# thanosDelatolas/eva-vos

Hardware: AMD Instinct MI355X
Metric: frames/sec STCN mask-propagate 480p 1-obj (higher is better)
Workload: dtype f32; 1 GPU; DAVIS-17-val-shaped 480x854 (padded 480x864) single-object STCN propagate: fresh engine, interact(mask,0), T=66 frames/video, mem_freq=5, top_k=50; one video per step per GPU; videos_per_gpu=38, streams_per_gpu=4, key_lookahead=0, clips=8 distinct synthetic clips (one per pooled engine), weights=synthetic recipe seed 0 (no checkpoints offline)

## Files before the change

### eva_vos_amd/_lib.py

```python
from __future__ import annotations

import ctypes as C
import os

import torch

_HERE = os.path.dirname(os.path.abspath(__file__))
LIB_PATH = os.environ.get("STCN_LIB") or os.path.join(_HERE, "libstcn_hip.so")

K_CLASSES = ("conv", "conv_reduce", "memread", "elementwise", "conv_n1", "other", "wino_input", "fusion_conv", "attention")


class WeightDesc(C.Structure):
    _fields_ = [("name", C.c_char_p), ("data", C.c_void_p), ("ndim", C.c_int32), ("shape", C.c_int64 * 4)]


class EngineOpts(C.Structure):
    _fields_ = [(n, C.c_int32) for n in ("lookahead", "decode_batch", "key_batch", "fuse_side")]


class ModelOpts(C.Structure):
    _fields_ = [("top_k", C.c_int32), ("km", C.c_float)]


# ... 24 lines not shown
    "stcn_engine_create_ex": (_I, [_P, _I, _I, _I, _I, _I, _P, _P, _P, _P, C.POINTER(EngineOpts), C.POINTER(_P)]),
    "stcn_engine_get_opts": (_I, [_P, C.POINTER(EngineOpts)]),
    "stcn_engine_destroy": (_I, [_P]),
    "stcn_engine_reset": (_I, [_P]),
    "stcn_engine_clone": (_I, [_P, _P, _P, _P, C.POINTER(_P)]),
    "stcn_interact": (_I, [_P, _P, _I, _I, _I]),
    "stcn_get_stats": (_I, [_P, C.POINTER(Stats)]),
    "stcn_get_flops": (_I, [_P, C.POINTER(_D)]),
    "stcn_last_conv_path": (C.c_char_p, []),
    "stcn_test_conv_trace": (_I, [_I]),
    "stcn_test_conv_trace_get": (C.c_char_p, []),
    "stcn_test_conv": (_I, [_P, _P, _P, _P, _P, _P] + [_I] * 11),
    "stcn_test_conv_ex": (_I, [_P, _P, _P, _P, _P, _P] + [_I] * 11 + [_P, _I, _L, _L, _L, _I, _L]),
    "stcn_test_conv_path": (_I, [_I] * 9 + [C.c_char_p, _I]),
    "stcn_test_conv_plan": (_I, [_I] * 9 + [C.POINTER(C.c_int32), _I, C.POINTER(_D)]),
    "stcn_test_sweep_plan": (_I, [_I, _I, _I, _I, C.POINTER(C.c_int32), _I, C.POINTER(C.c_int32)]),
    "stcn_test_encode_key": (_I, [_P, _P, _P, _I, _I, _P, _P, _P, _P, _P]),
    "stcn_test_encode_value": (_I, [_P, _P, _P, _P, _P, _I, _I, _I, _P]),
    "stcn_test_memory_read": (_I, [_P, _P, _P, _P, _I, _I, _I, _P, _P, _P]),
    "stcn_test_memory_read_k": (_I, [_P, _P, _P, _P, _I, _I, _I, _I, _P, _P, _P]),
    "stcn_test_memory_read_km": (_I, [_P, _P, _P, _P, _I, _I, _I, _I, _I, _I, _F, _P, _P, _P, _P]),
    "stcn_bench_memory_read": (_I, [_P, _P, _P, _P, _I, _I, _I, _I, _P, C.POINTER(_F), C.POINTER(C.c_int32)]),
    "stcn_bench_memory_read_k": (_I, [_P, _P, _P, _P, _I, _I, _I, _I, _I, _P, C.POINTER(_F), C.POINTER(C.c_int32)]),
    "stcn_bench_memory_read_km": (_I, [_P, _P, _P, _P, _I, _I, _I, _I, _I, _I, _F, _I, _P, C.POINTER(_F), C.POINTER(C.c_int32)]),
    "stcn_memread_plan": (_I, [_I, _I, C.POINTER(C.c_int32)]),
    "stcn_memread_scratch": (_I, [_I, C.POINTER(C.c_int64)]),
    "stcn_test_kernel": (_I, [C.c_char_p, _P, C.POINTER(_P), _I, C.POINTER(C.c_int64), _I, C.POINTER(_D), _I]),
    "stcn_test_fail_at": (_I, [_I]),
    "stcn_test_side_delay_us": (_I, [_I]),
    "stcn_test_decode": (_I, [_P, _P, _P, _P, _P, _P, _I, _I, _I, _P, _P]),
# ... 57 lines not shown
```

### eva_vos_amd/csrc/engine.cpp

```cpp
#include "engine.h"
#include "src_hash.h"

#include <algorithm>
#include <atomic>
#include <cmath>
#include <cstdarg>
#include <cstdio>
#include <cstdlib>
#include <cstring>
#include <map>
#include <mutex>
#include <unordered_map>
#include <utility>

namespace stcn {

static thread_local char g_err[512] = "";
void set_error(const char *fmt, ...) {
    va_list ap;
    va_start(ap, fmt);
    vsnprintf(g_err, sizeof(g_err), fmt, ap);
    va_end(ap);
}
const char *get_error() { return g_err; }

Knobs Knobs::from_env() {
    Knobs k;
    k.wino_min_cin = env_int("STCN_WINO_MIN_CIN", k.wino_min_cin);
    k.wino_ppw = env_int("STCN_WINO_PPW", k.wino_ppw);
    k.wino4_chunk_mb = env_int("STCN_WINO4_CHUNK_MB", k.wino4_chunk_mb);
    k.fusion_conv12 = env_int("STCN_FUSION_CONV12", k.fusion_conv12) != 0;
    k.fusion_wino = env_int("STCN_FUSION_WINO", k.fusion_wino) != 0;
    k.pw_chain = env_int("STCN_PW_CHAIN", k.pw_chain);
    return k;
}

void Prof::reset() {
    for (int i = 0; i < STCN_K_COUNT; ++i) { flops[i] = 0; bytes[i] = 0; exec_flops[i] = 0; launches[i] = 0; }
    hbm_conv_flops = hbm_conv_bytes = hbm_conv_ms = 0; hbm_conv_launches = 0;
    wino2_flops = wino4_flops = 0;
    for (auto &e : events) { pool.push_back(e.a); pool.push_back(e.b); }
    events.clear();
}
Prof::Ev &Prof::push_pair(int cls, bool hbm) {
    Ev e; e.cls = cls; e.hbm = hbm;
    for (hipEvent_t *p : {&e.a, &e.b}) {
        if (!pool.empty()) { *p = pool.back(); pool.pop_back(); }
        else (void)hipEventCreate(p);
// ... 74 lines not shown
int make_wino_fusion12(Model &m, ConvW &cw, const std::vector<float> &w) {
    if (!wants_wino_fusion12(cw)) return STCN_OK;
    std::vector<float> w16((size_t)32 * 9 * 16, 0.f), u((size_t)16 * 16 * 32);
    for (int n = 0; n < 32; ++n)
        for (int tap = 0; tap < 9; ++tap)
            for (int c = 0; c < 12; ++c) w16[((size_t)n * 9 + tap) * 16 + c] = w[(size_t)n * cw.Kp + tap * 12 + c];
    wino_transform_weights(w16.data(), 32, 16, 9 * 16, u.data());
    return upload(m, u, &cw.wino_u);
}

int make_wino4(Model &m, ConvW &cw, const std::vector<float> &w) {
    if (!wants_wino4(cw)) return STCN_OK;
    std::vector<float> u((size_t)36 * cw.cin_p * cw.cout);
    wino4_transform_weights(w.data(), cw.cout, cw.cin_p, cw.Kp, u.data());
    return upload(m, u, &cw.wino4_u);
}

static bool wino4_layer(const std::string &name) {
    if (name == "value_encoder.layer2.0.conv1" || name == "value_encoder.layer3.0.conv1") return false;
    if (name == "key_encoder.layer2.0.conv2" || name == "key_encoder.layer3.0.conv2") return false;
    static const bool key_f4 = env_on("STCN_WINO4_KEY");
    if (key_f4 && name.compare(0, 12, "key_encoder.") == 0 && name.size() > 6 && name.compare(name.size() - 6, 6, ".conv2") == 0) return true;
    static const bool kproj_f4 = env_on("STCN_WINO4_KEYPROJ");
    if (kproj_f4 && name == "key_proj.key_proj") return true;
    return name.compare(0, 8, "decoder.") == 0 || name == "key_comp" || name.compare(0, 20, "value_encoder.fuser.") == 0 ||
           name.compare(0, 19, "value_encoder.layer") == 0;
}

static std::vector<float> repack(const HostT &wt, const std::vector<float> &scale, int lo, int hi, const ConvW &cw) {
    const int cout = (int)wt.sh[0], cin = (int)wt.sh[1], kh = (int)wt.sh[2], kw = (int)wt.sh[3];
// ... 30 lines not shown
                const float sc = g[n] / std::sqrt(var[n] + 1e-5f);
                scale[n] = sc;
                bias[n] = (bias[n] - mu[n]) * sc + b[n];
            }
        }
        ConvW cw;
        cw.cout = cout; cw.cin = cin; cw.kh = kh; cw.kw = kw;
        cw.cin_p = (cin + 3) / 4 * 4;
        cw.K = kh * kw * cw.cin_p;
        cw.Kp = (cw.K + 31) / 32 * 32;
        const std::vector<float> w = repack(wt, scale, 0, cin, cw);
        int rc = upload(m, w, &cw.w);
        if (rc) return rc;
        rc = upload(m, bias, &cw.bias);
        if (rc) return rc;
        if ((rc = make_wino(m, cw, w)) || (rc = make_wino_fusion12(m, cw, w))) return rc;
        if (wino4_layer(pre) && (rc = make_wino4(m, cw, w))) return rc;
        cw.bias0 = bias[0];
        m.conv[pre] = cw;
        static const struct { const char *name; int c0; } splits[] = {
            {"decoder.compress.conv1", 512}, {"decoder.compress.downsample", 512},
            {"value_encoder.fuser.block1.conv1", 256}, {"value_encoder.fuser.block1.downsample", 256}};
        for (const auto &sp : splits) {
            if (pre != sp.name) continue;
            for (int part = 0; part < 2; ++part) {
                const int lo = part ? sp.c0 : 0, hi = part ? cin : sp.c0;
                ConvW pw;
                pw.cout = cout; pw.cin = hi - lo; pw.cin_p = hi - lo; pw.kh = kh; pw.kw = kw;
                pw.K = kh * kw * pw.cin_p; pw.Kp = (pw.K + 31) / 32 * 32;
                const std::vector<float> ww = repack(wt, scale, lo, hi, pw);
                std::vector<float> bb = part ? bias : std::vector<float>(cout, 0.f);
// ... 230 lines not shown
namespace {
struct ConvPathRec {
    ConvPlan plan{};
    char lit[96] = "";
};
thread_local ConvPathRec g_path;
thread_local char g_path_str[96] = "";
thread_local bool g_trace_on = false;
thread_local std::string g_trace;
}
const char *format_conv_path(const ConvPlan &pl, char *out, size_t n) {
    switch (pl.family) {
    case CONV_FUSION: snprintf(out, n, "%s", pl.fusion_wino ? "fusion_wino" : "fusion_direct"); break;
    case CONV_WINO4: snprintf(out, n, "wino4 chunks=%d%s", pl.w4.chunks, pl.reduce ? " +tail" : ""); break;
    case CONV_WINO2: snprintf(out, n, "wino2 ppw=%d splitk=%d", pl.ppw, pl.splitk); break;
    case CONV_DIRECT: snprintf(out, n, "%s%s splitk=%d", pl.variant, pl.tail ? " +tail" : "", pl.splitk); break;
    default: snprintf(out, n, "%s", "");
    }
    return out;
}
const char *last_conv_path() { return g_path.plan.family == CONV_LITERAL ? g_path.lit : format_conv_path(g_path.plan, g_path_str, sizeof(g_path_str)); }
void set_conv_path(const char *s) { g_path.plan.family = CONV_LITERAL; snprintf(g_path.lit, sizeof(g_path.lit), "%s", s); }
void conv_trace(int on) { g_trace_on = on != 0; if (on) g_trace.clear(); }
const char *conv_trace_get() { return g_trace.c_str(); }

int plan_conv(const Model &m, const Work &w, const std::string &name, const ConvArgs &a, ConvP &p, ConvPlan &pl) {
    auto it = m.conv.find(name);
    if (it == m.conv.end()) { set_error("missing conv '%s'", name.c_str()); return STCN_E_MISSING; }
    const ConvW &cw = it->second;
    const int B = a.B, H = a.H, W = a.W, c0 = a.c0, c1 = a.c1;
// ... 60 lines not shown
            eg[c] = w.prof->attach(cls, hbm_acc);
            if (c < pl.n_in) ei[c] = w.prof->attach(STCN_K_WINO_INPUT);
        }
        if (pl.reduce) er = w.prof->attach(STCN_K_CONV_REDUCE);
    }
    if (g_trace_on) { char b[96]; g_trace += name; g_trace += '='; g_trace += format_conv_path(pl, b, sizeof(b)); g_trace += '\n'; }
    switch (pl.family) {
    case CONV_FUSION: fusion_conv_launch(p, pl, s, eg[0]); break;
    case CONV_WINO4: wino4_launch(p, pl, w.wino_v, s, ei, eg, er); break;
    case CONV_WINO2: wino_launch(p, pl, w.wino_v, s, ei[0], eg[0], er); break;
    default: conv_launch(p, s, eg[0], er);
    }
    return launch_status(name.c_str());
}

#define RC(x) do { int rc_ = (x); if (rc_) return rc_; } while (0)

int encode_key(const Model &m, Work &w, hipStream_t s, const float *img4, const KeyOut &o, int B, long out_bs) {
    const Dims &d = w.d;
    const long obs = B > 1 ? out_bs : 0;
    const long ibs = obs ? obs : CONV_DENSE;
    RC(run_conv(m, w, s, "key_encoder.conv1", ConvArgs(img4, 4, B, d.nh, d.nw).strided(2).out(w.A).relu(0, 1)));
    { Scope sc(w.prof, STCN_K_ELEMWISE, s); maxpool3x3s2_launch(w.A, w.B, B, d.h2, d.w2, 64, s); }
    struct St { const char *name; int n, planes, stride; } stages[3] = {{"res2", 3, 64, 1}, {"layer2", 4, 128, 2}, {"layer3", 6, 256, 2}};
    int H = d.h4, W = d.w4, cin = 64;
    float *x = w.B;
    for (int si = 0; si < 3; ++si) {
        const St &st = stages[si];
        for (int i = 0; i < st.n; ++i) {
            const std::string p = std::string("key_encoder.") + st.name + "." + std::to_string(i);
            const int sd = i == 0 ? st.stride : 1;
            const int OH = H / sd, OW = W / sd;
            const float *idt = x;
            if (i == 0) { RC(run_conv(m, w, s, p + ".downsample.0", ConvArgs(x, cin, B, H, W).strided(sd).out(w.D))); idt = w.D; }
            RC(run_conv(m, w, s, p + ".conv1", ConvArgs(x, cin, B, H, W).out(w.C).relu(0, 1)));
            RC(run_conv(m, w, s, p + ".conv2", ConvArgs(w.C, st.planes, B, H, W).strided(sd).out(w.A).relu(0, 1)));
            float *dst = x;
            long dst_bs = 0;
// ... 48 lines not shown
    const ConvArgs in = ConvArgs(x0, c0, B, H, W, bs0).concat(x1, c1, bs1);
    const float *skip; long skip_bs;
    if (m.conv.count(p + ".downsample")) {
        RC(run_conv(m, w, s, p + ".downsample", ConvArgs(in).out(t2)));
        skip = t2; skip_bs = CONV_DENSE;
    } else { skip = x0; skip_bs = bs0; }
    RC(run_conv(m, w, s, p + ".conv1", ConvArgs(in).out(t1).relu(1, 1)));
    RC(run_conv(m, w, s, p + ".conv2", ConvArgs(t1, cw.cout, B, H, W).out(out, out_bs).residual(skip, skip_bs)));
    return STCN_OK;
}

int encode_value(const Model &m, Work &w, hipStream_t s, const float *img4, const float *f16, const float *masks,
                 long mask_stride, float *out, long out_bs, const float *vd, const float *vc) {
    const Dims &d = w.d;
    const int k = w.k;
    { Scope sc(w.prof, STCN_K_ELEMWISE, s); pack_value_input_launch(img4, masks, mask_stride, k, (int)d.npix, w.vin, s); }
    RC(run_conv(m, w, s, "value_encoder.conv1", ConvArgs(w.vin, 8, k, d.nh, d.nw).strided(2).out(w.C).relu(0, 1)));
    { Scope sc(w.prof, STCN_K_ELEMWISE, s); maxpool3x3s2_launch(w.C, w.B, k, d.h2, d.w2, 64, s); }
    int H = d.h4, W = d.w4, cin = 64;
    const int planes[3] = {64, 128, 256}, strides[3] = {1, 2, 2};
    for (int li = 0; li < 3; ++li)
        for (int i = 0; i < 2; ++i) {
            const std::string p = "value_encoder.layer" + std::to_string(li + 1) + "." + std::to_string(i);
            const int sd = i == 0 ? strides[li] : 1;
            const int OH = H / sd, OW = W / sd;
            const float *idt = w.B;
            if (m.conv.count(p + ".downsample.0")) {
                RC(run_conv(m, w, s, p + ".downsample.0", ConvArgs(w.B, cin, k, H, W).strided(sd).out(w.D)));
                idt = w.D;
            }
            RC(run_conv(m, w, s, p + ".conv1", ConvArgs(w.B, cin, k, H, W).strided(sd).out(w.C).relu(0, 1)));
            RC(run_conv(m, w, s, p + ".conv2", ConvArgs(w.C, planes[li], k, OH, OW).out(w.B).residual(idt).relu(0, 1)));
            H = OH; W = OW; cin = planes[li];
// ... 840 lines not shown
```

### eva_vos_amd/csrc/engine.h

```cpp
#pragma once
#include <hip/hip_runtime.h>

#include <deque>
#include <map>
#include <memory>
#include <set>
#include <string>
#include <vector>

#include "../../include/stcn_hip.h"
#include "kernels.h"

namespace stcn {

void set_error(const char *fmt, ...);
struct Model;
struct ConvW;
hipError_t pool_malloc(void **p, size_t bytes);
void pool_free(void *p);
void pool_release();
bool wants_wino(const ConvW &cw);
bool wants_wino4(const ConvW &cw);
bool wants_wino_fusion12(const ConvW &cw);
int make_wino(Model &m, ConvW &cw, const std::vector<float> &w_host);
int make_wino4(Model &m, ConvW &cw, const std::vector<float> &w_host);
int make_wino_fusion12(Model &m, ConvW &cw, const std::vector<float> &w_host);
#define HIPCHK(x)                                                                          \
    do {                                                                                   \
        hipError_t e_ = (x);                                                               \
        if (e_ != hipSuccess) {                                                            \
            set_error("%s:%d %s -> %s", __FILE__, __LINE__, #x, hipGetErrorString(e_));    \
            return STCN_E_HIP;                                                             \
        }                                                                                  \
    } while (0)

struct ConvW {
    float *w = nullptr, *bias = nullptr;
    float *wino_u = nullptr;
    float *wino4_u = nullptr;
    float bias0 = 0.f;
    int cout = 0, cin = 0, cin_p = 0, kh = 0, kw = 0, K = 0, Kp = 0;
};

struct Model {
    int device = 0;
    std::map<std::string, ConvW> conv;
    CbamW cbam{};
    bool has_prop = false;
    bool has_fuse = false;
    int top_k = MEMREAD_MAX_TOPK;
    float km = 0.f;
    int wino4_min_wg = 100;
    std::vector<void *> allocs;
    const ConvW &c(const std::string &name) const;
// ... 86 lines not shown
int plan_conv(const Model &m, const Work &w, const std::string &name, const ConvArgs &a, ConvP &p, ConvPlan &pl);
const char *format_conv_path(const ConvPlan &pl, char *out, size_t n);
int run_conv(const Model &m, Work &w, hipStream_t s, const std::string &name, const ConvArgs &a);
struct SweepGroup {
    int first;
    int t_lo;
    int G;
    bool inserts;
};
std::vector<SweepGroup> plan_sweep(int idx, int closest, int mem_freq, int cap);
constexpr int MAX_DECODE_GROUP = 8;
int encode_key(const Model &m, Work &w, hipStream_t s, const float *img4, const KeyOut &o, int B = 1, long out_bs = 0);
int encode_value(const Model &m, Work &w, hipStream_t s, const float *img4, const float *f16,
                 const float *masks, long mask_stride, float *out, long out_bs, const float *vd = nullptr,
                 const float *vc = nullptr);
int value_frame_parts(const Model &m, Work &w, hipStream_t s, const float *f16, float *vd, float *vc);
int decode(const Model &m, Work &w, hipStream_t s, const float *readout, const float *f16_thin,
           const float *s8, const float *s4, float *agg, long agg_stride, const float *dthin = nullptr,
           const float *cthin = nullptr, int G = 1, long slot_bs = 0, long agg_gs = 0);
int decode_logit4(const Model &m, Work &w, hipStream_t s, const float *readout, const float *f16_thin, const float *s8, const float *s4,
                  const float *dthin = nullptr, const float *cthin = nullptr, int G = 1, long slot_bs = 0);
int fusion_logit(const Model &m, Work &w, hipStream_t s, const float *img4, const float *prev,
                 const float *curr, const float *attn2, float nc, float nr, float *logit);

long stage_grow(long cap, long need);

}

struct stcn_model { stcn::Model m; };

// ... 45 lines not shown
```

### eva_vos_amd/csrc/hooks.cpp

```cpp
#include <algorithm>
#include <climits>
#include <cmath>
#include <cstdlib>
#include <cstring>
#include <string>
#include <vector>

#include "engine.h"

using namespace stcn;
#define RC(x) do { int rc_ = (x); if (rc_) return rc_; } while (0)

namespace {
struct TmpWork {
    Work w;
    int rc;
    TmpWork(int nh, int nw, int k) { rc = w.init(nh, nw, k); }
    ~TmpWork() { (void)hipDeviceSynchronize(); w.release(); }
};
struct DevBuf {
    float *p = nullptr;
    int alloc(size_t floats) { HIPCHK(hipMalloc((void **)&p, floats * 4)); return STCN_OK; }
    ~DevBuf() { if (p) { (void)hipDeviceSynchronize(); (void)hipFree(p); } }
};
// ... 152 lines not shown
int stcn_test_conv_plan(int B, int H, int W, int Cin, int Cout, int K, int stride, int flags, int splitk, int32_t *iv, int n, double *dv) {
    if (Cin % 4 || !iv || n < STCN_CONV_PLAN_INTS || !dv) { set_error("stcn_test_conv_plan: Cin%%4==0, STCN_CONV_PLAN_INTS ints and 2 doubles required"); return STCN_E_INVALID; }
    ConvP p;
    ConvPlan pl;
    RC(plan_test_conv(B, H, W, Cin, Cout, K, stride, flags, splitk, p, pl));
    const bool w2 = pl.family == CONV_WINO2, w4 = pl.family == CONV_WINO4, direct = pl.family == CONV_DIRECT;
    const WinoGeom g = w2 || w4 ? pl.geo : WinoGeom{};
    const W4Plan q = w4 ? pl.w4 : W4Plan{};
    const int32_t v[STCN_CONV_PLAN_INTS] = {
        pl.family, pl.splitk, pl.ppw, pl.tail, pl.n_in, pl.n_gemm, pl.reduce,
        g.TH, g.TW, g.Mt, g.Mt_pad, g.KB, w2 ? pl.w2.kb_per_split : 0,
        q.mb, q.tiles_m, q.tiles_n, q.grid, q.full_wg, q.pieces, q.per, q.chunks, q.tm_per_chunk,
        direct ? p.tile_big : 0, direct ? p.rem_full : 0, direct ? p.rem_split : 0, direct ? p.rem_per : 0, direct ? p.chain : 0};
    for (int i = 0; i < STCN_CONV_PLAN_INTS; ++i) iv[i] = v[i];
    dv[0] = (double)pl.v_floats; dv[1] = pl.fl_exec;
    return STCN_OK;
}

int stcn_bench_conv(void *stream, int B, int H, int W, int Cin, int Cout, int KH, int KW, int stride, int pad, int splitk,
                    int iters, float *avg_ms, double *flops_per_launch) {
    hipStream_t s = (hipStream_t)stream;
    (void)pad;
    ConvW cw = test_convw(Cin, Cout, KH, KW);
    const int OH = (H + 2 * (KH / 2) - KH) / stride + 1, OW = (W + 2 * (KW / 2) - KW) / stride + 1;
    DevBuf x, wt, b, y;
    RC(x.alloc((size_t)B * H * W * Cin)); RC(wt.alloc((size_t)Cout * cw.Kp)); RC(b.alloc(Cout));
    RC(y.alloc((size_t)B * OH * OW * Cout));
    std::vector<float> h((size_t)B * H * W * Cin);
    unsigned st = 12345u;
    auto rnd = [&]() { st = st * 1664525u + 1013904223u; return ((st >> 8) & 0xffff) / 32768.f - 1.f; };
// ... 326 lines not shown
```

### eva_vos_amd/csrc/kernels.h

```cpp
#pragma once
#include <hip/hip_runtime.h>
#include <stdint.h>

#include <cstdlib>

#include "../../include/stcn_hip.h"

namespace stcn {

struct FastDiv {
    unsigned magic, shift, d;
};
static inline FastDiv fastdiv_make(unsigned d) {
    FastDiv f{0, 0, d};
    if (d <= 1) return f;
    unsigned s = 0;
    while ((1ull << s) < d) ++s;
    f.magic = (unsigned)(((1ull << (31 + s)) / d) + 1);
    f.shift = s - 1;
    return f;
}
#if defined(__HIPCC__)
__device__ __forceinline__ int fastdiv(int x, const FastDiv f) {
    return f.d <= 1 ? x : (int)(__umulhi((unsigned)x, f.magic) >> f.shift);
// ... 2 lines not shown
    const int q8 = nblk >> 3, r8 = nblk & 7, xcd = bid & 7;
    return (xcd < r8 ? xcd * (q8 + 1) : r8 * (q8 + 1) + (xcd - r8) * q8) + (bid >> 3);
}
#endif

static inline int env_int(const char *name, int dflt) { const char *e = getenv(name); return e ? atoi(e) : dflt; }
static inline bool env_on(const char *name, bool dflt = true) { return env_int(name, dflt) != 0; }
int device_cus();

struct Knobs {
    int wino_min_cin = 128;
    int wino_ppw = 0;
    int wino4_chunk_mb = 160;
    int fusion_conv12 = 0;
    int fusion_wino = 1;
    int pw_chain = 2;
    static Knobs from_env();
};

struct ConvP {
    const float *x0, *x1;
    int c0, c1;
    long bs0, bs1;
    unsigned x0_bytes, x1_bytes, w_bytes;
    int B, H, W;
    int OH, OW;
    int KH, KW, stride, pad;
    int Cin;
    int M, N;
    int K, Kp;
// ... 11 lines not shown
    const float *wino_u;
    const float *wino4_u;
    FastDiv fd_ohw, fd_ow;
    FastDiv fd_cin, fd_kw;
    int pointwise;
    int affine_out;
    int tile_big;
    int panel;
    int chain;
    Knobs kn;
};
constexpr int W4_MAX_CHUNKS = 16;
struct WinoGeom { int TH, TW, Mt, Mt_pad, KB; };
struct W2Plan { int tiles_n, ntile, kb_per_split; };
struct W4Plan { int tiles_m, tiles_n, mb, grid, full_wg, pieces, per, chunks, tm_per_chunk, judge_wg; };
enum ConvFamily { CONV_LITERAL = 0, CONV_FUSION = 1, CONV_WINO4 = 2, CONV_WINO2 = 3, CONV_DIRECT = 4 };
struct ConvPlan {
    int family = CONV_LITERAL;
    bool fusion_wino = false;
    WinoGeom geo{};
    W4Plan w4{};
    W2Plan w2{};
    int splitk = 1;
    int ppw = 0;
    const char *variant = "";
    bool tail = false;
    size_t v_floats = 0;
    int n_in = 0, n_gemm = 1;
    bool reduce = false;
    double fl = 0;
    double fl_exec = 0;
// ... 5 lines not shown
void wino_launch(const ConvP &p, const ConvPlan &pl, float *V, hipStream_t s, hipEvent_t *ev_in = nullptr, hipEvent_t *ev_gemm = nullptr,
                 hipEvent_t *ev_red = nullptr);
void wino_transform_weights(const float *w, int N, int Cin, int Kp, float *U);
#ifndef W4_MIN_CIN
#define W4_MIN_CIN 64
#endif
bool wino4_plan(const ConvP &p, int min_wg, size_t v_cap, size_t slab_floats, ConvPlan &pl);
void wino4_launch(const ConvP &p, const ConvPlan &pl, float *V, hipStream_t s, hipEvent_t *const *ev_in = nullptr,
                  hipEvent_t *const *ev_gemm = nullptr, hipEvent_t *ev_red = nullptr);
void wino4_transform_weights(const float *w, int N, int Cin, int Kp, float *U);
bool wino_enabled();
int wino4_mode();

bool fusion_conv_plan(const ConvP &p, ConvPlan &pl);
void fusion_conv_launch(const ConvP &p, const ConvPlan &pl, hipStream_t s, hipEvent_t *ev_gemm = nullptr);

void conv_n1_launch(const float *x, const float *w, float bias, float *y, int B, int H, int W, int C,
                    int KH, int relu_in, hipStream_t s);

void maxpool3x3s2_launch(const float *x, float *y, int B, int H, int W, int C, hipStream_t s);
void pack_image_launch(const float *img_chw, float *out, int H, int W, int nh, int nw, int lw, int lh,
                       hipStream_t s);
void pack_value_input_launch(const float *img4, const float *masks, long mask_stride, int k, int npix,
                             float *out, hipStream_t s);
void upsample2x_add_launch(const float *x, const float *skip, float *u, int B, int h, int w, int C,
                           hipStream_t s, long skip_bs = 0, int skip_bmod = 0);
void up4_sigmoid_aggregate_launch(const float *logit4, int k, int h4, int w4, float *agg,
                                  long agg_stride, hipStream_t s, long obj_stride = 0, int G = 1, long logit_gs = 0, long agg_gs = 0);
void up4_sigmoid_launch(const float *logit4, int k, int h4, int w4, float *prob, hipStream_t s);
void aggregate_wbg_launch(const float *prob, int k, long npix, int keep_bg, int hard, float *out, hipStream_t s);
// ... 69 lines not shown
```

### include/stcn_hip.h

```cpp
#ifndef STCN_HIP_H
#define STCN_HIP_H

#include <stddef.h>
#include <stdint.h>

#ifdef __cplusplus
extern "C" {
#endif

#define STCN_OK            0
#define STCN_E_INVALID    -1
#define STCN_E_MISSING    -2
#define STCN_E_HIP        -3
#define STCN_E_STATE      -4

#define STCN_MAX_OBJECTS  32

typedef struct stcn_model  stcn_model;
typedef struct stcn_engine stcn_engine;

typedef struct {
    const char  *name;
    const float *data;
    int32_t      ndim;
// ... 56 lines not shown
int stcn_fusion_model_create(int device, const stcn_weight_desc *fuse, int n_fuse, stcn_model **out);
int stcn_test_transpose(void *stream, const float *src, float *dst, int B, int R, int C, long ld, long planes_bs, int to_rows);


int stcn_test_conv(void *stream, const float *x, const float *w, const float *bias, const float *res,
                   float *y, int B, int H, int W, int Cin, int Cout, int KH, int KW, int stride,
                   int pad, int flags, int splitk);

int stcn_test_conv_ex(void *stream, const float *x, const float *w, const float *bias, const float *res,
                      float *y, int B, int H, int W, int Cin, int Cout, int KH, int KW, int stride,
                      int pad, int flags, int splitk, const float *x1, int c1, long bs0, long bs1, long res_bs, int res_bmod, long y_bs);

int stcn_test_conv_path(int B, int H, int W, int Cin, int Cout, int K, int stride, int flags, int splitk, char *out, int n);
#define STCN_CONV_PLAN_INTS 27
int stcn_test_conv_plan(int B, int H, int W, int Cin, int Cout, int K, int stride, int flags, int splitk, int32_t *iv, int n, double *dv);
const char *stcn_last_conv_path(void);
int stcn_test_sweep_plan(int idx, int closest, int mem_freq, int cap, int32_t *out, int n, int32_t *count);
int stcn_test_conv_trace(int on);
const char *stcn_test_conv_trace_get(void);

int stcn_test_kernel(const char *name, void *stream, void *const *ptrs, int nptr, const int64_t *iv, int ni, const double *fv, int nf);

int stcn_test_encode_key(const stcn_model *m, void *stream, const float *img, int nh, int nw,
                         float *k16, float *f16_thin, float *f16, float *f8, float *f4);

int stcn_test_encode_value(const stcn_model *m, void *stream, const float *img, const float *f16,
                           const float *masks, int k, int nh, int nw, float *out);

int stcn_test_memory_read(void *stream, const float *mk, const float *mv, const float *qk,
                          int N, int Q, int k, int32_t *topk_idx, float *topk_w, float *readout);
// ... 59 lines not shown
```

Measured before the change: 807.1 frames/s.

## Fuse 7x7 stride-2 stem conv, ReLU and 3x3 maxpool into one MFMA kernel

Adds a dedicated stem kernel for the key and value encoders. It computes the 7x7 stride-2 conv with fp32 MFMA over an LDS-staged input patch, then applies bias, ReLU and the 3x3 stride-2 maxpool inside the same tile before writing the quarter-resolution output. For the value encoder it also builds the 5-channel input (image, mask, sum of the other objects' masks) on the fly, so the separate pack kernel goes away. This removes the full-size intermediate conv output, the separate maxpool launch and its memory round trips. The cost is recomputing overlapping halo pixels per tile and a large, complex register/LDS-heavy kernel; unsupported shapes fall back to the old path.

```diff
diff --git a/eva_vos_amd/_lib.py b/eva_vos_amd/_lib.py
--- a/eva_vos_amd/_lib.py
+++ b/eva_vos_amd/_lib.py
@@ -62,6 +62,9 @@
     "stcn_test_conv_ex": (_I, [_P, _P, _P, _P, _P, _P] + [_I] * 11 + [_P, _I, _L, _L, _L, _I, _L]),
     "stcn_test_conv_path": (_I, [_I] * 9 + [C.c_char_p, _I]),
     "stcn_test_conv_plan": (_I, [_I] * 9 + [C.POINTER(C.c_int32), _I, C.POINTER(_D)]),
+    "stcn_test_stem_pool": (_I, [_P, _P, _P, _I, _P, _P, _I, _I, _I, _P]),
+    "stcn_test_stem_plan": (_I, [_I, _I, _I, _I, C.POINTER(C.c_int32), _I, C.POINTER(_D)]),
+    "stcn_test_stem_repack": (_I, [_I, _P, _P]),
     "stcn_test_sweep_plan": (_I, [_I, _I, _I, _I, C.POINTER(C.c_int32), _I, C.POINTER(C.c_int32)]),
     "stcn_test_encode_key": (_I, [_P, _P, _P, _I, _I, _P, _P, _P, _P, _P]),
     "stcn_test_encode_value": (_I, [_P, _P, _P, _P, _P, _I, _I, _I, _P]),
diff --git a/eva_vos_amd/csrc/engine.cpp b/eva_vos_amd/csrc/engine.cpp
--- a/eva_vos_amd/csrc/engine.cpp
+++ b/eva_vos_amd/csrc/engine.cpp
@@ -32,6 +32,7 @@
     k.fusion_conv12 = env_int("STCN_FUSION_CONV12", k.fusion_conv12) != 0;
     k.fusion_wino = env_int("STCN_FUSION_WINO", k.fusion_wino) != 0;
     k.pw_chain = env_int("STCN_PW_CHAIN", k.pw_chain);
+    k.stem = env_int("STCN_STEM", k.stem) != 0;
     return k;
 }
 
@@ -136,6 +137,13 @@
     std::vector<float> u((size_t)36 * cw.cin_p * cw.cout);
     wino4_transform_weights(w.data(), cw.cout, cw.cin_p, cw.Kp, u.data());
     return upload(m, u, &cw.wino4_u);
+}
+
+int make_stem(Model &m, ConvW &cw, const std::vector<float> &w) {
+    if (cw.kh != 7 || cw.kw != 7 || cw.cout != 64 || (cw.cin != 3 && cw.cin != 5)) return STCN_OK;
+    std::vector<float> sw((size_t)stem_weight_floats(cw.cin));
+    stem_repack_weights(cw.cin, w.data(), cw.Kp, cw.cin_p, sw.data());
+    return upload(m, sw, &cw.stem_w);
 }
 
 static bool wino4_layer(const std::string &name) {
@@ -196,7 +204,7 @@
         if (rc) return rc;
         rc = upload(m, bias, &cw.bias);
         if (rc) return rc;
-        if ((rc = make_wino(m, cw, w)) || (rc = make_wino_fusion12(m, cw, w))) return rc;
+        if ((rc = make_wino(m, cw, w)) || (rc = make_wino_fusion12(m, cw, w)) || (rc = make_stem(m, cw, w))) return rc;
         if (wino4_layer(pre) && (rc = make_wino4(m, cw, w))) return rc;
         cw.bias0 = bias[0];
         m.conv[pre] = cw;
@@ -457,6 +465,7 @@
     case CONV_FUSION: snprintf(out, n, "%s", pl.fusion_wino ? "fusion_wino" : "fusion_direct"); break;
     case CONV_WINO4: snprintf(out, n, "wino4 chunks=%d%s", pl.w4.chunks, pl.reduce ? " +tail" : ""); break;
     case CONV_WINO2: snprintf(out, n, "wino2 ppw=%d splitk=%d", pl.ppw, pl.splitk); break;
+    case CONV_STEM: snprintf(out, n, "%s", "stem_pool"); break;
     case CONV_DIRECT: snprintf(out, n, "%s%s splitk=%d", pl.variant, pl.tail ? " +tail" : "", pl.splitk); break;
     default: snprintf(out, n, "%s", "");
     }
@@ -547,14 +556,51 @@
     return launch_status(name.c_str());
 }
 
+int run_stem(const Model &m, Work &w, hipStream_t s, const std::string &name, const float *img4, const float *masks, long mask_stride, int B,
+             float *out, bool *done) {
+    *done = false;
+    if (!w.kn.stem) return STCN_OK;
+    auto it = m.conv.find(name);
+    if (it == m.conv.end()) { set_error("missing conv '%s'", name.c_str()); return STCN_E_MISSING; }
+    const ConvW &cw = it->second;
+    StemPlan sp;
+    if (!cw.stem_w || !cw.bias || (cw.cin == 5) != (masks != nullptr) || !stem_pool_plan(cw.cin, B, w.d.nh, w.d.nw, masks ? mask_stride : 0, sp)) return STCN_OK;
+    ConvPlan &pl = g_path.plan;
+    pl = ConvPlan{};
+    pl.family = CONV_STEM; pl.fl = sp.fl; pl.fl_exec = sp.fl_exec;
+    hipEvent_t *ev = nullptr;
+    if (w.prof) {
+        const double in = masks ? (double)w.d.npix * (4 + B) : (double)B * w.d.npix * 4;
+        const double bytes = 4.0 * (in + 64.0 * 49 * cw.cin + (double)B * w.d.hw4 * 64);
+        const int cls = w.conv_cls;
+        const bool hbm_acc = pl.fl / bytes < 157.3e12 / 8.0e12 && cls == STCN_K_CONV;
+        w.prof->bytes[cls] += bytes;
+        w.prof->flops[cls] += pl.fl;
+        w.prof->exec_flops[cls] += pl.fl_exec;
+        if (hbm_acc) { w.prof->hbm_conv_bytes += bytes; w.prof->hbm_conv_flops += pl.fl; }
+        ev = w.prof->attach(cls, hbm_acc);
+    }
+    if (g_trace_on) { g_trace += name; g_trace += "=stem_pool\n"; }
+    StemP p{};
+    p.img4 = img4; p.img_batched = masks ? 0 : 1; p.masks = masks; p.mask_stride = mask_stride; p.k = masks ? B : 0;
+    p.w = cw.stem_w; p.bias = cw.bias; p.B = B; p.nh = w.d.nh; p.nw = w.d.nw; p.out = out;
+    stem_pool_launch(p, sp, s, ev);
+    *done = true;
+    return launch_status(name.c_str());
+}
+
 #define RC(x) do { int rc_ = (x); if (rc_) return rc_; } while (0)
 
 int encode_key(const Model &m, Work &w, hipStream_t s, const float *img4, const KeyOut &o, int B, long out_bs) {
     const Dims &d = w.d;
     const long obs = B > 1 ? out_bs : 0;
     const long ibs = obs ? obs : CONV_DENSE;
-    RC(run_conv(m, w, s, "key_encoder.conv1", ConvArgs(img4, 4, B, d.nh, d.nw).strided(2).out(w.A).relu(0, 1)));
-    { Scope sc(w.prof, STCN_K_ELEMWISE, s); maxpool3x3s2_launch(w.A, w.B, B, d.h2, d.w2, 64, s); }
+    bool stem = false;
+    RC(run_stem(m, w, s, "key_encoder.conv1", img4, nullptr, 0, B, w.B, &stem));
+    if (!stem) {
+        RC(run_conv(m, w, s, "key_encoder.conv1", ConvArgs(img4, 4, B, d.nh, d.nw).strided(2).out(w.A).relu(0, 1)));
+        { Scope sc(w.prof, STCN_K_ELEMWISE, s); maxpool3x3s2_launch(w.A, w.B, B, d.h2, d.w2, 64, s); }
+    }
     struct St { const char *name; int n, planes, stride; } stages[3] = {{"res2", 3, 64, 1}, {"layer2", 4, 128, 2}, {"layer3", 6, 256, 2}};
     int H = d.h4, W = d.w4, cin = 64;
     float *x = w.B;
@@ -633,9 +679,13 @@
                  long mask_stride, float *out, long out_bs, const float *vd, const float *vc) {
     const Dims &d = w.d;
     const int k = w.k;
-    { Scope sc(w.prof, STCN_K_ELEMWISE, s); pack_value_input_launch(img4, masks, mask_stride, k, (int)d.npix, w.vin, s); }
-    RC(run_conv(m, w, s, "value_encoder.conv1", ConvArgs(w.vin, 8, k, d.nh, d.nw).strided(2).out(w.C).relu(0, 1)));
-    { Scope sc(w.prof, STCN_K_ELEMWISE, s); maxpool3x3s2_launch(w.C, w.B, k, d.h2, d.w2, 64, s); }
+    bool stem = false;
+    RC(run_stem(m, w, s, "value_encoder.conv1", img4, masks, mask_stride, k, w.B, &stem));
+    if (!stem) {
+        { Scope sc(w.prof, STCN_K_ELEMWISE, s); pack_value_input_launch(img4, masks, mask_stride, k, (int)d.npix, w.vin, s); }
+        RC(run_conv(m, w, s, "value_encoder.conv1", ConvArgs(w.vin, 8, k, d.nh, d.nw).strided(2).out(w.C).relu(0, 1)));
+        { Scope sc(w.prof, STCN_K_ELEMWISE, s); maxpool3x3s2_launch(w.C, w.B, k, d.h2, d.w2, 64, s); }
+    }
     int H = d.h4, W = d.w4, cin = 64;
     const int planes[3] = {64, 128, 256}, strides[3] = {1, 2, 2};
     for (int li = 0; li < 3; ++li)
diff --git a/eva_vos_amd/csrc/engine.h b/eva_vos_amd/csrc/engine.h
--- a/eva_vos_amd/csrc/engine.h
+++ b/eva_vos_amd/csrc/engine.h
@@ -38,6 +38,7 @@
     float *w = nullptr, *bias = nullptr;
     float *wino_u = nullptr;
     float *wino4_u = nullptr;
+    float *stem_w = nullptr;
     float bias0 = 0.f;
     int cout = 0, cin = 0, cin_p = 0, kh = 0, kw = 0, K = 0, Kp = 0;
 };
@@ -154,6 +155,9 @@
 int encode_value(const Model &m, Work &w, hipStream_t s, const float *img4, const float *f16,
                  const float *masks, long mask_stride, float *out, long out_bs, const float *vd = nullptr,
                  const float *vc = nullptr);
+int run_stem(const Model &m, Work &w, hipStream_t s, const std::string &name, const float *img4, const float *masks, long mask_stride, int B,
+             float *out, bool *done);
+int make_stem(Model &m, ConvW &cw, const std::vector<float> &w_host);
 int value_frame_parts(const Model &m, Work &w, hipStream_t s, const float *f16, float *vd, float *vc);
 int decode(const Model &m, Work &w, hipStream_t s, const float *readout, const float *f16_thin,
            const float *s8, const float *s4, float *agg, long agg_stride, const float *dthin = nullptr,
diff --git a/eva_vos_amd/csrc/hooks.cpp b/eva_vos_amd/csrc/hooks.cpp
--- a/eva_vos_amd/csrc/hooks.cpp
+++ b/eva_vos_amd/csrc/hooks.cpp
@@ -190,6 +190,47 @@
         direct ? p.tile_big : 0, direct ? p.rem_full : 0, direct ? p.rem_split : 0, direct ? p.rem_per : 0, direct ? p.chain : 0};
     for (int i = 0; i < STCN_CONV_PLAN_INTS; ++i) iv[i] = v[i];
     dv[0] = (double)pl.v_floats; dv[1] = pl.fl_exec;
+    return STCN_OK;
+}
+
+int stcn_test_stem_pool(void *stream, const float *img4, const float *masks, int k, const float *wgt, const float *bias, int B, int nh, int nw,
+                        float *out) {
+    if (!img4 || !wgt || !bias || !out || (masks ? k < 1 : B < 1)) { set_error("stcn_test_stem_pool: img4, w, bias, out and B >= 1 (k >= 1 with masks) required"); return STCN_E_INVALID; }
+    hipStream_t s = (hipStream_t)stream;
+    const int cr = masks ? 5 : 3, cp = masks ? 8 : 4, nb = masks ? k : B;
+    StemPlan sp;
+    if (!stem_pool_plan(cr, nb, nh, nw, masks ? (long)nh * nw : 0, sp)) { set_error("stcn_test_stem_pool: %dx%d (batch %d) is not a shape of the stem kernel", nh, nw, nb); return STCN_E_INVALID; }
+    std::vector<float> hw((size_t)64 * 49 * cp), sw((size_t)stem_weight_floats(cr));
+    HIPCHK(hipStreamSynchronize(s));
+    HIPCHK(hipMemcpy(hw.data(), wgt, hw.size() * 4, hipMemcpyDeviceToHost));
+    stem_repack_weights(cr, hw.data(), 49 * cp, cp, sw.data());
+    DevBuf dw;
+    RC(dw.alloc(sw.size()));
+    HIPCHK(hipMemcpy(dw.p, sw.data(), sw.size() * 4, hipMemcpyHostToDevice));
+    StemP p{};
+    p.img4 = img4; p.img_batched = masks ? 0 : 1; p.masks = masks; p.mask_stride = (long)nh * nw; p.k = masks ? k : 0;
+    p.w = dw.p; p.bias = bias; p.B = nb; p.nh = nh; p.nw = nw; p.out = out;
+    stem_pool_launch(p, sp, s);
+    RC(launch_status("stem_pool"));
+    HIPCHK(hipStreamSynchronize(s));
+    HIPCHK(hipGetLastError());
+    return STCN_OK;
+}
+
+int stcn_test_stem_plan(int cr, int B, int nh, int nw, int32_t *iv, int n, double *dv) {
+    if ((cr != 3 && cr != 5) || !iv || n < STCN_STEM_PLAN_INTS || !dv) { set_error("stcn_test_stem_plan: cr 3 or 5, STCN_STEM_PLAN_INTS ints and 2 doubles required"); return STCN_E_INVALID; }
+    StemPlan sp;
+    stem_pool_plan(cr, B, nh, nw, cr == 5 ? (long)nh * nw : 0, sp);
+    const int32_t v[STCN_STEM_PLAN_INTS] = {sp.eligible, sp.patch_h, sp.patch_w, sp.tiles_y, sp.tiles_x, sp.grid, sp.threads, sp.lds_bytes, sp.steps, sp.mp};
+    for (int i = 0; i < STCN_STEM_PLAN_INTS; ++i) iv[i] = v[i];
+    dv[0] = sp.fl; dv[1] = sp.fl_exec;
+    return STCN_OK;
+}
+
+int stcn_test_stem_repack(int cr, const float *w, float *out) {
+    if ((cr != 3 && cr != 5) || !w || !out) { set_error("stcn_test_stem_repack: cr 3 or 5, w and out required"); return STCN_E_INVALID; }
+    const int cp = cr == 3 ? 4 : 8;
+    stem_repack_weights(cr, w, 49 * cp, cp, out);
     return STCN_OK;
 }
 
diff --git a/eva_vos_amd/csrc/kernels.h b/eva_vos_amd/csrc/kernels.h
--- a/eva_vos_amd/csrc/kernels.h
+++ b/eva_vos_amd/csrc/kernels.h
@@ -40,6 +40,7 @@
     int wino4_chunk_mb = 160;
     int fusion_conv12 = 0;
     int fusion_wino = 1;
+    int stem = 1;
     int pw_chain = 2;
     static Knobs from_env();
 };
@@ -81,7 +82,7 @@
 struct WinoGeom { int TH, TW, Mt, Mt_pad, KB; };
 struct W2Plan { int tiles_n, ntile, kb_per_split; };
 struct W4Plan { int tiles_m, tiles_n, mb, grid, full_wg, pieces, per, chunks, tm_per_chunk, judge_wg; };
-enum ConvFamily { CONV_LITERAL = 0, CONV_FUSION = 1, CONV_WINO4 = 2, CONV_WINO2 = 3, CONV_DIRECT = 4 };
+enum ConvFamily { CONV_LITERAL = 0, CONV_FUSION = 1, CONV_WINO4 = 2, CONV_WINO2 = 3, CONV_DIRECT = 4, CONV_STEM = 5 };
 struct ConvPlan {
     int family = CONV_LITERAL;
     bool fusion_wino = false;
@@ -117,6 +118,20 @@
 
 bool fusion_conv_plan(const ConvP &p, ConvPlan &pl);
 void fusion_conv_launch(const ConvP &p, const ConvPlan &pl, hipStream_t s, hipEvent_t *ev_gemm = nullptr);
+
+struct StemP {
+    const float *img4; int img_batched;
+    const float *masks; long mask_stride; int k;
+    const float *w;
+    const float *bias;
+    int B, nh, nw;
+    float *out;
+};
+struct StemPlan { int eligible, cr, patch_h, patch_w, tiles_y, tiles_x, grid, threads, lds_bytes, steps, mp; double fl, fl_exec; };
+bool stem_pool_plan(int cr, int B, int nh, int nw, long mask_stride, StemPlan &pl);
+void stem_pool_launch(const StemP &p, const StemPlan &pl, hipStream_t s, hipEvent_t *ev = nullptr);
+int stem_weight_floats(int cr);
+void stem_repack_weights(int cr, const float *w, int Kp, int cin_p, float *out);
 
 void conv_n1_launch(const float *x, const float *w, float bias, float *y, int B, int H, int W, int C,
                     int KH, int relu_in, hipStream_t s);
diff --git a/eva_vos_amd/csrc/stem_conv.hip b/eva_vos_amd/csrc/stem_conv.hip
--- /dev/null
+++ b/eva_vos_amd/csrc/stem_conv.hip
@@ -0,0 +1,277 @@
+#include <hip/hip_ext.h>
+
+#include <type_traits>
+#include <utility>
+
+#include "kernels.h"
+
+namespace stcn {
+
+typedef float f32x4 __attribute__((ext_vector_type(4)));
+typedef float f32x16 __attribute__((ext_vector_type(16)));
+
+namespace {
+constexpr unsigned OOB = 0x80000000u;
+constexpr int SP_PH = 8, SP_PW = 14;
+constexpr int SP_CH = 2 * SP_PH + 1, SP_CW = 2 * SP_PW + 1, SP_NCV = SP_CH * SP_CW;
+constexpr int SP_MB = (SP_NCV + 31) / 32;
+constexpr int SP_WAVES = 8, SP_RM = SP_MB / SP_WAVES, SP_THREADS = 64 * SP_WAVES;
+constexpr int SP_ROWS = 2 * (SP_CH - 1) + 7, SP_COLS = 2 * (SP_CW - 1) + 7;
+constexpr int SP_HW = (SP_COLS + 1) / 2, SP_RS = 2 * SP_HW;
+constexpr int SP_PLANE = SP_ROWS * SP_RS;
+constexpr int SP_NPOS = SP_ROWS * SP_RS, SP_NIT = (SP_NPOS + SP_THREADS - 1) / SP_THREADS;
+constexpr int SP_EXF = SP_MB * 32 * 32;
+
+template <int CR>
+struct StemK {
+    static constexpr int NTERM = CR == 3 ? 150 : 246, NSTEP = NTERM / 2, MP = NSTEP + 1, NG = MP / 4;
+    static constexpr int tap(int i) { return CR == 3 ? 2 * (i / 6) + (i & 1) : i / 5; }
+    static constexpr int slot(int i) { return CR == 3 ? (i % 6) / 2 : i % 5; }
+    static constexpr int chan(int s) { return CR == 3 ? s : (s == 0 ? 0 : (s == 1 ? 4 : s - 1)); }
+    static constexpr int off(int i) {
+        const int t = tap(i) > 48 ? 48 : tap(i), kh = t / 7, kw = t % 7;
+        return slot(i) * SP_PLANE + kh * SP_RS + (kw & 1) * SP_HW + (kw >> 1);
+    }
+    struct Tab { int n; int d[8]; int cls[128]; };
+    static constexpr Tab make() {
+        Tab t{};
+        for (int m = 0; m < NSTEP; ++m) {
+            const int dm = off(2 * m + 1) - off(2 * m);
+            int c = 0;
+            while (c < t.n && t.d[c] != dm) ++c;
+            if (c == t.n) t.d[t.n++] = dm;
+            t.cls[m] = c;
+        }
+        return t;
+    }
+};
+template <int CR> struct StemTab { static constexpr typename StemK<CR>::Tab tab = StemK<CR>::make(); };
+static_assert(StemTab<3>::tab.n <= 5 && StemTab<5>::tab.n <= 5, "bases per row block");
+static_assert(StemK<3>::MP % 8 == 4 && StemK<5>::MP % 8 == 4, "weight rows: an odd number of 16-byte slots (conflict-free ds_read_b128)");
+
+template <int I, int N, class F>
+__device__ __forceinline__ void sfor(F &&f) {
+    if constexpr (I < N) {
+        f(std::integral_constant<int, I>{});
+        sfor<I + 1, N>(f);
+    }
+}
+}
+
+struct StemKP {
+    const float *img4; unsigned img_bytes; int img_bs_pix;
+    const float *masks; unsigned mask_bytes; int mask_stride; int k;
+    const float *w; const float *bias; float *out;
+    int nh, nw, h4, w4, tiles_x, tiles_img;
+};
+
+template <int CR>
+__global__ __launch_bounds__(SP_THREADS, CR == 3 ? 4 : 2) void stem_pool_kernel(const StemKP p) {
+    using K = StemK<CR>;
+    constexpr int NC = StemTab<CR>::tab.n;
+    constexpr int WF = 64 * 2 * K::MP;
+    constexpr int NWI = (WF / 4 + SP_THREADS - 1) / SP_THREADS;
+    extern __shared__ __attribute__((aligned(16))) float smem[];
+    float *const wl = smem, *const patch = smem + WF, *const ex = smem;
+    const int t = threadIdx.x, lane = t & 63, l31 = lane & 31, h = lane >> 5;
+    const int wave = __builtin_amdgcn_readfirstlane(t >> 6);
+    const int bid = xcd_contiguous_block((int)blockIdx.x, (int)gridDim.x);
+    const int b = bid / p.tiles_img, rem = bid - b * p.tiles_img;
+    const int ty = rem / p.tiles_x, tx = rem - ty * p.tiles_x;
+    const int py0 = ty * SP_PH, px0 = tx * SP_PW;
+    const int iy0 = 4 * py0 - 5, ix0 = 4 * px0 - 5;
+
+    const __amdgpu_buffer_rsrc_t ri = __builtin_amdgcn_make_buffer_rsrc(const_cast<float *>(p.img4), 0, p.img_bytes, 0x00020000);
+    const __amdgpu_buffer_rsrc_t rw = __builtin_amdgcn_make_buffer_rsrc(const_cast<float *>(p.w), 0, WF * 4, 0x00020000);
+    const __amdgpu_buffer_rsrc_t rm =
+        __builtin_amdgcn_make_buffer_rsrc(const_cast<float *>(CR == 5 ? p.masks : p.img4), 0, CR == 5 ? p.mask_bytes : p.img_bytes, 0x00020000);
+    f32x4 im[SP_NIT], wr[NWI];
+    float me[SP_NIT], ot[SP_NIT];
+    int pixo[SP_NIT];
+#pragma unroll
+    for (int i = 0; i < SP_NIT; ++i) {
+        const int idx = t + SP_THREADS * i;
+        const int pr = idx / SP_RS, pc = idx - pr * SP_RS;
+        const int gy = iy0 + pr, gx = ix0 + pc;
+        const bool ok = idx < SP_NPOS && (unsigned)gy < (unsigned)p.nh && (unsigned)gx < (unsigned)p.nw;
+        pixo[i] = ok ? gy * p.nw + gx : -1;
+        im[i] = __builtin_bit_cast(f32x4, __builtin_amdgcn_raw_buffer_load_b128(ri, ok ? (unsigned)(b * p.img_bs_pix + pixo[i]) * 16u : OOB, 0, 0));
+        me[i] = 0.f; ot[i] = 0.f;
+        if (CR == 5) me[i] = __builtin_bit_cast(float, __builtin_amdgcn_raw_buffer_load_b32(rm, ok ? (unsigned)(b * p.mask_stride + pixo[i]) * 4u : OOB, 0, 0));
+    }
+#pragma unroll
+    for (int i = 0; i < NWI; ++i)
+        wr[i] = __builtin_bit_cast(f32x4, __builtin_amdgcn_raw_buffer_load_b128(rw, (unsigned)(t + SP_THREADS * i) * 16u, 0, 0));
+    float bv[2];
+    bv[0] = p.bias[l31]; bv[1] = p.bias[32 + l31];
+    if (CR == 5 && p.k > 1) {
+        for (int j = 0; j < p.k; ++j) {
+            if (j == b) continue;
+#pragma unroll
+            for (int i = 0; i < SP_NIT; ++i)
+                ot[i] += __builtin_bit_cast(float, __builtin_amdgcn_raw_buffer_load_b32(rm, pixo[i] >= 0 ? (unsigned)(j * p.mask_stride + pixo[i]) * 4u : OOB, 0, 0));
+        }
+    }
+#pragma unroll
+    for (int i = 0; i < SP_NIT; ++i) {
+        const int idx = t + SP_THREADS * i;
+        const int pr = idx / SP_RS, pc = idx - pr * SP_RS;
+        float *dst = patch + pr * SP_RS + (pc & 1) * SP_HW + (pc >> 1);
+        if (idx < SP_NPOS) {
+            if (CR == 3) {
+                dst[0] = im[i].x; dst[SP_PLANE] = im[i].y; dst[2 * SP_PLANE] = im[i].z;
+            } else {
+                dst[0] = im[i].x; dst[SP_PLANE] = ot[i]; dst[2 * SP_PLANE] = im[i].y; dst[3 * SP_PLANE] = im[i].z; dst[4 * SP_PLANE] = me[i];
+            }
+        }
+    }
+#pragma unroll
+    for (int i = 0; i < NWI; ++i) {
+        const int idx = t + SP_THREADS * i;
+        if (idx < WF / 4) *reinterpret_cast<f32x4 *>(wl + 4 * idx) = wr[i];
+    }
+    const float *vb[NC][SP_RM];
+#pragma unroll
+    for (int a = 0; a < SP_RM; ++a) {
+        const int q = min((wave * SP_RM + a) * 32 + l31, SP_NCV - 1);
+        const int cy = q / SP_CW, cx = q - cy * SP_CW;
+        const float *base = patch + cy * 2 * SP_RS + cx;
+        sfor<0, NC>([&](auto cc) {
+            constexpr int c = decltype(cc)::value, d = StemTab<CR>::tab.d[c];
+            vb[c][a] = base + h * d;
+        });
+    }
+    const float *wb = wl + (l31 * 2 + h) * K::MP;
+    f32x16 acc[SP_RM][2];
+#pragma unroll
+    for (int a = 0; a < SP_RM; ++a)
+#pragma unroll
+        for (int nb = 0; nb < 2; ++nb)
+#pragma unroll
+            for (int e = 0; e < 16; ++e) acc[a][nb][e] = 0.f;
+    __syncthreads();
+
+    f32x4 fb[2][2];
+    float fa[2][4][SP_RM];
+    auto fread = [&](auto gc, auto sc) {
+        constexpr int g = decltype(gc)::value, set = decltype(sc)::value;
+        fb[set][0] = *reinterpret_cast<const f32x4 *>(wb + 4 * g);
+        fb[set][1] = *reinterpret_cast<const f32x4 *>(wb + 64 * K::MP + 4 * g);
+        sfor<0, 4>([&](auto jc) {
+            constexpr int j = decltype(jc)::value, m = 4 * g + j;
+            if constexpr (m < K::NSTEP) {
+                constexpr int c = StemTab<CR>::tab.cls[m], o = K::off(2 * m);
+#pragma unroll
+                for (int a = 0; a < SP_RM; ++a) fa[set][j][a] = vb[c][a][o];
+            }
+        });
+    };
+    fread(std::integral_constant<int, 0>{}, std::integral_constant<int, 0>{});
+    sfor<0, K::NG>([&](auto gc) {
+        constexpr int g = decltype(gc)::value, set = g & 1;
+        if constexpr (g + 1 < K::NG) fread(std::integral_constant<int, g + 1>{}, std::integral_constant<int, set ^ 1>{});
+        __builtin_amdgcn_sched_barrier(0);
+        sfor<0, 4>([&](auto jc) {
+            constexpr int j = decltype(jc)::value, m = 4 * g + j;
+            if constexpr (m < K::NSTEP) {
+#pragma unroll
+                for (int a = 0; a < SP_RM; ++a)
+#pragma unroll
+                    for (int nb = 0; nb < 2; ++nb)
+                        acc[a][nb] = __builtin_amdgcn_mfma_f32_32x32x2f32(fa[set][j][a], fb[set][nb][j], acc[a][nb], 0, 0, 0);
+            }
+        });
+        __builtin_amdgcn_sched_barrier(0);
+    });
+
+    const int rlo = py0 == 0 ? 1 : 0, clo = px0 == 0 ? 1 : 0;
+#pragma unroll
+    for (int nb = 0; nb < 2; ++nb) {
+        __syncthreads();
+#pragma unroll
+        for (int a = 0; a < SP_RM; ++a) {
+            const int q0 = (wave * SP_RM + a) * 32 + 4 * h;
+#pragma unroll
+            for (int r = 0; r < 16; ++r) {
+                const int q = q0 + (r & 3) + 8 * (r >> 2);
+                ex[q * 32 + l31] = fmaxf(acc[a][nb][r] + bv[nb], 0.f);
+            }
+        }
+        __syncthreads();
+#pragma unroll
+        for (int i = 0; i < (SP_PH * SP_PW * 8 + SP_THREADS - 1) / SP_THREADS; ++i) {
+            const int idx = t + SP_THREADS * i;
+            const int pp = idx >> 3, cq = idx & 7, ppy = pp / SP_PW, ppx = pp - ppy * SP_PW;
+            if (idx < SP_PH * SP_PW * 8) {
+                f32x4 v[9];
+#pragma unroll
+                for (int dy = 0; dy < 3; ++dy)
+#pragma unroll
+                    for (int dx = 0; dx < 3; ++dx) {
+                        const int cr = max(2 * ppy + dy, rlo), cc = max(2 * ppx + dx, clo);
+                        v[dy * 3 + dx] = *reinterpret_cast<const f32x4 *>(ex + (cr * SP_CW + cc) * 32 + 4 * cq);
+                    }
+                f32x4 mx = v[0];
+#pragma unroll
+                for (int e = 1; e < 9; ++e) { mx.x = fmaxf(mx.x, v[e].x); mx.y = fmaxf(mx.y, v[e].y); mx.z = fmaxf(mx.z, v[e].z); mx.w = fmaxf(mx.w, v[e].w); }
+                const int gy = py0 + ppy, gx = px0 + ppx;
+                if (gy < p.h4 && gx < p.w4) *reinterpret_cast<f32x4 *>(p.out + (((long)b * p.h4 + gy) * p.w4 + gx) * 64 + nb * 32 + 4 * cq) = mx;
+            }
+        }
+    }
+}
+
+int stem_weight_floats(int cr) { return cr == 3 ? 64 * 2 * StemK<3>::MP : 64 * 2 * StemK<5>::MP; }
+
+template <int CR>
+static void repack_t(const float *w, int Kp, int cin_p, float *out) {
+    using K = StemK<CR>;
+    for (int n = 0; n < 64; ++n)
+        for (int hh = 0; hh < 2; ++hh)
+            for (int m = 0; m < K::MP; ++m) {
+                const int i = 2 * m + hh;
+                float v = 0.f;
+                if (m < K::NSTEP && K::tap(i) < 49) v = w[(size_t)n * Kp + K::tap(i) * cin_p + K::chan(K::slot(i))];
+                out[((size_t)n * 2 + hh) * K::MP + m] = v;
+            }
+}
+void stem_repack_weights(int cr, const float *w, int Kp, int cin_p, float *out) {
+    if (cr == 3) repack_t<3>(w, Kp, cin_p, out); else repack_t<5>(w, Kp, cin_p, out);
+}
+
+bool stem_pool_plan(int cr, int B, int nh, int nw, long mask_stride, StemPlan &pl) {
+    pl = StemPlan{};
+    pl.cr = cr;
+    if ((cr != 3 && cr != 5) || B < 1 || nh < 16 || nw < 16 || nh % 16 || nw % 16) return false;
+    if ((long)B * nh * nw * 16 >= (1L << 31)) return false;
+    if (cr == 5 && (mask_stride < (long)nh * nw || ((long)(B - 1) * mask_stride + (long)nh * nw) * 4 >= (1L << 31))) return false;
+    const int h4 = nh / 4, w4 = nw / 4;
+    pl.patch_h = SP_PH; pl.patch_w = SP_PW;
+    pl.tiles_y = (h4 + SP_PH - 1) / SP_PH; pl.tiles_x = (w4 + SP_PW - 1) / SP_PW;
+    if ((long)B * pl.tiles_y * pl.tiles_x >= (1L << 31)) return false;
+    pl.grid = B * pl.tiles_y * pl.tiles_x;
+    pl.threads = SP_THREADS;
+    pl.steps = cr == 3 ? StemK<3>::NSTEP : StemK<5>::NSTEP;
+    pl.mp = pl.steps + 1;
+    const int wp = (64 * 2 * pl.mp + cr * SP_PLANE) * 4;
+    pl.lds_bytes = wp > SP_EXF * 4 ? wp : SP_EXF * 4;
+    pl.fl = 2.0 * B * (nh / 2) * (double)(nw / 2) * 64 * 49 * cr;
+    pl.fl_exec = (double)pl.grid * SP_MB * 2 * pl.steps * (2.0 * 32 * 32 * 2);
+    pl.eligible = 1;
+    return true;
+}
+
+void stem_pool_launch(const StemP &a, const StemPlan &pl, hipStream_t s, hipEvent_t *ev) {
+    StemKP p{};
+    p.img4 = a.img4; p.img_bs_pix = a.img_batched ? a.nh * a.nw : 0;
+    p.img_bytes = (unsigned)((long)(a.img_batched ? a.B : 1) * a.nh * a.nw * 16);
+    p.masks = a.masks; p.mask_stride = (int)a.mask_stride; p.k = a.k;
+    p.mask_bytes = a.masks ? (unsigned)(((long)(a.k - 1) * a.mask_stride + (long)a.nh * a.nw) * 4) : 0u;
+    p.w = a.w; p.bias = a.bias; p.out = a.out;
+    p.nh = a.nh; p.nw = a.nw; p.h4 = a.nh / 4; p.w4 = a.nw / 4;
+    p.tiles_x = pl.tiles_x; p.tiles_img = pl.tiles_x * pl.tiles_y;
+    if (pl.cr == 3) launch(stem_pool_kernel<3>, dim3((unsigned)pl.grid), dim3(SP_THREADS), (size_t)pl.lds_bytes, s, ev, p);
+    else launch(stem_pool_kernel<5>, dim3((unsigned)pl.grid), dim3(SP_THREADS), (size_t)pl.lds_bytes, s, ev, p);
+}
+
+}
diff --git a/include/stcn_hip.h b/include/stcn_hip.h
--- a/include/stcn_hip.h
+++ b/include/stcn_hip.h
@@ -94,6 +94,11 @@
 int stcn_test_conv_path(int B, int H, int W, int Cin, int Cout, int K, int stride, int flags, int splitk, char *out, int n);
 #define STCN_CONV_PLAN_INTS 27
 int stcn_test_conv_plan(int B, int H, int W, int Cin, int Cout, int K, int stride, int flags, int splitk, int32_t *iv, int n, double *dv);
+int stcn_test_stem_pool(void *stream, const float *img4, const float *masks, int k, const float *w, const float *bias, int B, int nh, int nw,
+                        float *out);
+#define STCN_STEM_PLAN_INTS 10
+int stcn_test_stem_plan(int cr, int B, int nh, int nw, int32_t *iv, int n, double *dv);
+int stcn_test_stem_repack(int cr, const float *w, float *out);
 const char *stcn_last_conv_path(void);
 int stcn_test_sweep_plan(int idx, int closest, int mem_freq, int cap, int32_t *out, int n, int32_t *count);
 int stcn_test_conv_trace(int on);
```

Measured after the change: 817.2 frames/s (median of 4 runs). Within noise of the previous version (+1.3%).
